# shuwang127/SRCNN_Cpp

Hardware: AMD Instinct MI355X
Metric: SRCNN Y-channel Mpixels/sec (higher is better)
Workload: dtype f32

## Files before the change

srcnn_cpp_amd/csrc/srcnn_pipeline.hip:

```cpp
#include "srcnn_image.h"

#pragma clang fp contract(off)

namespace srcnn {

__device__ __forceinline__ int descale14(int x) { return (x + (1 << 13)) >> 14; }
__device__ __forceinline__ uint8_t sat8(int v) { return (uint8_t)min(max(v, 0), 255); }

__global__ __launch_bounds__(256) void bgr2ycrcb_kernel(const uint8_t *__restrict__ bgr, long stride, int w, int h,
                                                        uint8_t *__restrict__ planes, long pstride, long ppitch)
{
    const int c = blockIdx.x * 256 + threadIdx.x, r = blockIdx.y;
    if (c >= w || r >= h) return;
    const uint8_t *p = bgr + (long)r * stride + 3L * c;
    const int B = p[0], G = p[1], R = p[2];
    const int Y = descale14(B * 1868 + G * 9617 + R * 4899);
    const long o = (long)r * pstride + c;
    planes[o] = sat8(Y);
    planes[ppitch + o] = sat8(descale14((R - Y) * 11682 + (128 << 14)));
    planes[2 * ppitch + o] = sat8(descale14((B - Y) * 9241 + (128 << 14)));
}

__global__ __launch_bounds__(256) void ycrcb2bgr_kernel(const uint8_t *__restrict__ yp, long ystride,
                                                        const uint8_t *__restrict__ crcb, long pstride, long ppitch,
                                                        int w, int h, uint8_t *__restrict__ bgr, long stride)
{
    const int c = blockIdx.x * 256 + threadIdx.x, r = blockIdx.y;
    if (c >= w || r >= h) return;
    const int Y = yp[(long)r * ystride + c];
    const long o = (long)r * pstride + c;
    const int Cr = crcb[o] - 128, Cb = crcb[ppitch + o] - 128;
    uint8_t *p = bgr + (long)r * stride + 3L * c;
    p[0] = sat8(Y + descale14(Cb * 29049));
    p[1] = sat8(Y + descale14(Cb * -5636 + Cr * -11698));
    p[2] = sat8(Y + descale14(Cr * 22987));
}

__device__ __forceinline__ unsigned vresize_px(int h0, int h1, int h2, int h3, int b0, int b1, int b2, int b3, bool simd)
{
    if (simd) {
        const float sc = 1.0f / (2048.0f * 2048.0f);
        float r = __fmul_rn((float)h3, (float)b3 * sc);
        r = __fadd_rn(__fmul_rn((float)h2, (float)b2 * sc), r);
        r = __fadd_rn(__fmul_rn((float)h1, (float)b1 * sc), r);
        r = __fadd_rn(__fmul_rn((float)h0, (float)b0 * sc), r);
        return sat8(__float2int_rn(r));
    }
    return sat8((h0 * b0 + h1 * b1 + h2 * b2 + h3 * b3 + (1 << 21)) >> 22);
}

__global__ __launch_bounds__(256) void resize_cubic_kernel(const uint8_t *__restrict__ src, long sstride, long spitch,
                                                           int sw, int sh, uint8_t *__restrict__ dst, long dstride,
                                                           long dpitch, int dw, int dh,
                                                           const int *__restrict__ xofs, const short *__restrict__ alpha,
                                                           const int *__restrict__ yofs, const short *__restrict__ beta)
{
    const int dx = blockIdx.x * 256 + threadIdx.x, dy = blockIdx.y;
    if (dx >= dw || dy >= dh) return;
    const uint8_t *s = src + (long)blockIdx.z * spitch;
    const int x0 = xofs[dx] - 1, y0 = yofs[dy] - 1;
    int a[4], xs[4];
#pragma unroll
    for (int k = 0; k < 4; ++k) {
        a[k] = alpha[4 * dx + k];
        xs[k] = min(max(x0 + k, 0), sw - 1);
    }
    int hs[4];
#pragma unroll
    for (int ky = 0; ky < 4; ++ky) {
        const uint8_t *row = s + (long)min(max(y0 + ky, 0), sh - 1) * sstride;
        int t = 0;
#pragma unroll
        for (int kx = 0; kx < 4; ++kx) t += row[xs[kx]] * a[kx];
        hs[ky] = t;
    }
    const short *b = beta + 4 * dy;
    dst[(long)blockIdx.z * dpitch + (long)dy * dstride + dx] =
        (uint8_t)vresize_px(hs[0], hs[1], hs[2], hs[3], b[0], b[1], b[2], b[3], dx < dw - dw % 8);
}


__global__ __launch_bounds__(256) void resize_cubic_tiled_kernel(const uint8_t *__restrict__ src, long sstride,
                                                                 long spitch, int sw, int sh,
                                                                 uint8_t *__restrict__ dst, long dstride, long dpitch,
                                                                 int dw, int dh, const int *__restrict__ xofs,
                                                                 const short *__restrict__ alpha,
                                                                 const int *__restrict__ yofs,
                                                                 const short *__restrict__ beta)
{
    __shared__ int hbuf[RMAX][256];
    __shared__ uint8_t sbuf[RMAX][SMAX];
    const int dx0 = blockIdx.x * 256, dx = dx0 + threadIdx.x;
    const int dy0 = blockIdx.y * RT, dy1 = min(dy0 + RT, dh);
    const uint8_t *s = src + (long)blockIdx.z * spitch;
    const int r_lo = yofs[dy0] - 1, r_hi = yofs[dy1 - 1] + 2;
    const int c_lo = xofs[dx0] - 1, c_hi = xofs[min(dx0 + 255, dw - 1)] + 2;
    const int ncol = c_hi - c_lo + 1, nrow = r_hi - r_lo + 1;
    for (int e = threadIdx.x; e < nrow * ncol; e += 256) {
        const int rr = e / ncol, cc = e - rr * ncol;
        sbuf[rr][cc] = s[(long)min(max(r_lo + rr, 0), sh - 1) * sstride + min(max(c_lo + cc, 0), sw - 1)];
    }
    __syncthreads();
    const int dxc = min(dx, dw - 1);
    const int x0 = xofs[dxc] - 1 - c_lo;
    int a[4];
#pragma unroll
    for (int k = 0; k < 4; ++k) a[k] = alpha[4 * dxc + k];
    for (int rr = 0; rr < nrow; ++rr) {
        int t = 0;
#pragma unroll
        for (int k = 0; k < 4; ++k) t += sbuf[rr][x0 + k] * a[k];
        hbuf[rr][threadIdx.x] = t;
    }
    if (dx >= dw) return;
    for (int dy = dy0; dy < dy1; ++dy) {
        const int j = yofs[dy] - 1 - r_lo;
        const short *b = beta + 4 * dy;
        dst[(long)blockIdx.z * dpitch + (long)dy * dstride + dx] =
            (uint8_t)vresize_px(hbuf[j][threadIdx.x], hbuf[j + 1][threadIdx.x], hbuf[j + 2][threadIdx.x],
                                hbuf[j + 3][threadIdx.x], b[0], b[1], b[2], b[3], dx < dw - dw % 8);
    }
}

__device__ __forceinline__ unsigned vpass4(const float (*hbuf)[256], int tx, int j, const short *__restrict__ b, int dx, int dw)
{
    typedef float f32x4 __attribute__((ext_vector_type(4)));
    f32x4 h[4];
#pragma unroll
    for (int k = 0; k < 4; ++k) h[k] = *reinterpret_cast<const f32x4 *>(&hbuf[j + k][4 * tx]);
    unsigned r = 0;
    if (dx + 3 < dw - dw % 8) {
        const float sc = 1.0f / (2048.0f * 2048.0f);
        const float b0 = (float)b[0] * sc, b1 = (float)b[1] * sc, b2 = (float)b[2] * sc, b3 = (float)b[3] * sc;
#pragma unroll
        for (int c = 0; c < 4; ++c) {
            float v = __fmul_rn(h[3][c], b3);
            v = __fadd_rn(__fmul_rn(h[2][c], b2), v);
            v = __fadd_rn(__fmul_rn(h[1][c], b1), v);
            v = __fadd_rn(__fmul_rn(h[0][c], b0), v);
            r |= (unsigned)sat8(__float2int_rn(v)) << (8 * c);
        }
    } else {
#pragma unroll
        for (int c = 0; c < 4; ++c)
            r |= vresize_px((int)h[0][c], (int)h[1][c], (int)h[2][c], (int)h[3][c], b[0], b[1], b[2], b[3], dx + c < dw - dw % 8) << (8 * c);
    }
    return r;
}


__global__ __launch_bounds__(256) void resize_cubic_tiled4_kernel(const uint8_t *__restrict__ src, long sstride,
                                                                  long spitch, int sw, int sh,
                                                                  uint8_t *__restrict__ dst, long dstride, long dpitch,
                                                                  int dw, int dh, const int *__restrict__ xofs,
                                                                  const short *__restrict__ alpha,
                                                                  const int *__restrict__ yofs,
                                                                  const short *__restrict__ beta)
{
    __shared__ __attribute__((aligned(16))) float hbuf[RMAX4][256];
    __shared__ uint8_t sbuf[RMAX4][SMAX];
    const int tid = threadIdx.x;
    const int dx0 = blockIdx.x * 256;
    const int dy0 = blockIdx.y * RT4, dy1 = min(dy0 + RT4, dh);
    const uint8_t *s = src + (long)blockIdx.z * spitch;
    const int r_lo = yofs[dy0] - 1, r_hi = yofs[dy1 - 1] + 2;
    const int c_lo = xofs[dx0] - 1, c_hi = xofs[min(dx0 + 255, dw - 1)] + 2;
    const int ncol = c_hi - c_lo + 1, nrow = r_hi - r_lo + 1;
    for (int e = tid; e < nrow * ncol; e += 256) {
        const int rr = e / ncol, cc = e - rr * ncol;
        sbuf[rr][cc] = s[(long)min(max(r_lo + rr, 0), sh - 1) * sstride + min(max(c_lo + cc, 0), sw - 1)];
    }
    __syncthreads();
    {
        const int dxc = min(dx0 + tid, dw - 1);
        const int x0 = xofs[dxc] - 1 - c_lo;
        int a[4];
#pragma unroll
        for (int k = 0; k < 4; ++k) a[k] = alpha[4 * dxc + k];
        for (int rr = 0; rr < nrow; ++rr) {
            int t = 0;
#pragma unroll
            for (int k = 0; k < 4; ++k) t += sbuf[rr][x0 + k] * a[k];
            hbuf[rr][tid] = (float)t;
        }
    }
    __syncthreads();
    const int tx = tid & 63, ty = tid >> 6;
    const int dx = dx0 + 4 * tx;
    if (dx >= dw) return;
    for (int r = 0; r < RPT; ++r) {
        const int dy = dy0 + RPT * ty + r;
        if (dy >= dy1) break;
        const unsigned v = vpass4(hbuf, tx, yofs[dy] - 1 - r_lo, beta + 4 * dy, dx, dw);
        uint8_t *o = dst + (long)blockIdx.z * dpitch + (long)dy * dstride + dx;
        if (dx + 3 < dw) *reinterpret_cast<unsigned *>(o) = v;
        else
            for (int c = 0; c < 4 && dx + c < dw; ++c) o[c] = (uint8_t)(v >> (8 * c));
    }
}

__device__ __forceinline__ int bgr_to_comp(const uint8_t *px, int comp)
{
    const int B = px[0], G = px[1], R = px[2];
    const int Y = descale14(B * 1868 + G * 9617 + R * 4899);
    if (comp == 0) return sat8(Y);
    if (comp == 1) return sat8(descale14((R - Y) * 11682 + (128 << 14)));
    return sat8(descale14((B - Y) * 9241 + (128 << 14)));
}

struct TileGeom {
    int dx0, dy0, dy1, r_lo, c_lo, ncol, nrow;
};

__device__ __forceinline__ void stage_and_hpass(const uint8_t *__restrict__ bgr, long stride, int sw, int sh, int dw, int comp,
                                                const TileGeom &g, const int *__restrict__ xofs,
                                                const short *__restrict__ alpha, uint8_t (*sbuf)[SMAX], float (*hbuf)[256])
{
    const int tid = threadIdx.x;
    for (int e = tid; e < g.nrow * g.ncol; e += 256) {
        const int rr = e / g.ncol, cc = e - rr * g.ncol;
        sbuf[rr][cc] = (uint8_t)bgr_to_comp(bgr + (long)min(max(g.r_lo + rr, 0), sh - 1) * stride + 3L * min(max(g.c_lo + cc, 0), sw - 1), comp);
    }
    __syncthreads();
    const int dxc = min(g.dx0 + tid, dw - 1);
    const int x0 = xofs[dxc] - 1 - g.c_lo;
    int a[4];
#pragma unroll
    for (int k = 0; k < 4; ++k) a[k] = alpha[4 * dxc + k];
    for (int rr = 0; rr < g.nrow; ++rr) {
        int t = 0;
#pragma unroll
        for (int k = 0; k < 4; ++k) t += sbuf[rr][x0 + k] * a[k];
        hbuf[rr][tid] = (float)t;
    }
    __syncthreads();
}

__device__ __forceinline__ TileGeom tile_geom(int dw, int dh, const int *__restrict__ xofs, const int *__restrict__ yofs)
{
    TileGeom g;
    g.dx0 = blockIdx.x * 256;
    g.dy0 = blockIdx.y * RT4;
    g.dy1 = min(g.dy0 + RT4, dh);
    g.r_lo = yofs[g.dy0] - 1;
    g.c_lo = xofs[g.dx0] - 1;
    g.ncol = xofs[min(g.dx0 + 255, dw - 1)] + 2 - g.c_lo + 1;
    g.nrow = yofs[g.dy1 - 1] + 2 - g.r_lo + 1;
    return g;
}

__global__ __launch_bounds__(256) void bgr_to_y_resized_kernel(const uint8_t *__restrict__ bgr, long stride, int sw, int sh,
                                                               uint8_t *__restrict__ dst, long dstride, int dw, int dh,
                                                               const int *__restrict__ xofs, const short *__restrict__ alpha,
                                                               const int *__restrict__ yofs, const short *__restrict__ beta)
{
    __shared__ __attribute__((aligned(16))) float hbuf[RMAX4][256];
    __shared__ uint8_t sbuf[RMAX4][SMAX];
    const TileGeom g = tile_geom(dw, dh, xofs, yofs);
    stage_and_hpass(bgr, stride, sw, sh, dw, 0, g, xofs, alpha, sbuf, hbuf);
    const int tx = threadIdx.x & 63, ty = threadIdx.x >> 6, dx = g.dx0 + 4 * tx;
    if (dx >= dw) return;
    for (int r = 0; r < RPT; ++r) {
        const int dy = g.dy0 + RPT * ty + r;
        if (dy >= g.dy1) break;
        const unsigned v = vpass4(hbuf, tx, yofs[dy] - 1 - g.r_lo, beta + 4 * dy, dx, dw);
        uint8_t *o = dst + (long)dy * dstride + dx;
        if (dx + 3 < dw) *reinterpret_cast<unsigned *>(o) = v;
        else
            for (int c = 0; c < 4 && dx + c < dw; ++c) o[c] = (uint8_t)(v >> (8 * c));
    }
}

__global__ __launch_bounds__(256) void resize_merge_kernel(const uint8_t *__restrict__ bgr, long stride, int sw, int sh,
                                                           const uint8_t *__restrict__ ysr, long ystride,
                                                           uint8_t *__restrict__ out, long ostride, int dw, int dh,
                                                           const int *__restrict__ xofs, const short *__restrict__ alpha,
                                                           const int *__restrict__ yofs, const short *__restrict__ beta)
{
    __shared__ __attribute__((aligned(16))) float hbuf[RMAX4][256];
    __shared__ uint8_t sbuf[RMAX4][SMAX];
    const TileGeom g = tile_geom(dw, dh, xofs, yofs);
    const int tx = threadIdx.x & 63, ty = threadIdx.x >> 6, dx = g.dx0 + 4 * tx;
    unsigned crcb[2][RPT];
#pragma unroll
    for (int pl = 0; pl < 2; ++pl) {
        if (pl) __syncthreads();
        stage_and_hpass(bgr, stride, sw, sh, dw, 1 + pl, g, xofs, alpha, sbuf, hbuf);
#pragma unroll
        for (int r = 0; r < RPT; ++r) {
            const int dy = min(g.dy0 + RPT * ty + r, g.dy1 - 1);
            crcb[pl][r] = vpass4(hbuf, tx, yofs[dy] - 1 - g.r_lo, beta + 4 * dy, min(dx, dw - 1), dw);
        }
    }
    if (dx >= dw) return;
#pragma unroll
    for (int r = 0; r < RPT; ++r) {
        const int dy = g.dy0 + RPT * ty + r;
        if (dy >= g.dy1) break;
        const uint8_t *yrow = ysr + (long)dy * ystride + dx;
        uint8_t *o = out + (long)dy * ostride + 3L * dx;
        const bool vec = dx + 3 < dw;
        unsigned yv = 0;
        if (vec) yv = *reinterpret_cast<const unsigned *>(yrow);
        else
            for (int c = 0; c < 4 && dx + c < dw; ++c) yv |= (unsigned)yrow[c] << (8 * c);
        uint8_t px[12];
#pragma unroll
        for (int c = 0; c < 4; ++c) {
            const int Y = (yv >> (8 * c)) & 255, Cr = (int)((crcb[0][r] >> (8 * c)) & 255) - 128,
                      Cb = (int)((crcb[1][r] >> (8 * c)) & 255) - 128;
            px[3 * c + 0] = sat8(Y + descale14(Cb * 29049));
            px[3 * c + 1] = sat8(Y + descale14(Cb * -5636 + Cr * -11698));
            px[3 * c + 2] = sat8(Y + descale14(Cr * 22987));
        }
        if (vec) {
            unsigned *o4 = reinterpret_cast<unsigned *>(o);
#pragma unroll
            for (int q = 0; q < 3; ++q)
                o4[q] = px[4 * q] | (px[4 * q + 1] << 8) | (px[4 * q + 2] << 16) | ((unsigned)px[4 * q + 3] << 24);
        } else {
            for (int c = 0; c < 4 && dx + c < dw; ++c)
                for (int q = 0; q < 3; ++q) o[3 * c + q] = px[3 * c + q];
        }
    }
}

bool fused_pipeline_ok(int sw, int sh, int dw, int dh, const void *y_hi, long ystride, const void *out, long ostride)
{
    const bool aligned = ((reinterpret_cast<uintptr_t>(y_hi) | (uintptr_t)ystride | reinterpret_cast<uintptr_t>(out) | (uintptr_t)ostride) & 3) == 0;
    return resize_variant(sw, sh, dw, dh, aligned) == RESIZE_TILED4;
}

hipError_t launch_bgr_to_y_resized(const uint8_t *bgr, long stride, int sw, int sh, uint8_t *dst, long dstride, int dw, int dh,
                                   const int *xofs, const short *alpha, const int *yofs, const short *beta, hipStream_t st)
{
    hipLaunchKernelGGL(bgr_to_y_resized_kernel, dim3((dw + 255) / 256, (dh + RT4 - 1) / RT4), dim3(256), 0, st, bgr, stride, sw,
                       sh, dst, dstride, dw, dh, xofs, alpha, yofs, beta);
    return hipGetLastError();
}

hipError_t launch_resize_merge(const uint8_t *bgr, long stride, int sw, int sh, const uint8_t *ysr, long ystride, uint8_t *out,
                               long ostride, int dw, int dh, const int *xofs, const short *alpha, const int *yofs,
                               const short *beta, hipStream_t st)
{
    hipLaunchKernelGGL(resize_merge_kernel, dim3((dw + 255) / 256, (dh + RT4 - 1) / RT4), dim3(256), 0, st, bgr, stride, sw, sh,
                       ysr, ystride, out, ostride, dw, dh, xofs, alpha, yofs, beta);
    return hipGetLastError();
}

__global__ __launch_bounds__(256) void copy_rows_kernel(uint8_t *__restrict__ dst, long dstride, const uint8_t *__restrict__ src,
                                                        long sstride, int width)
{
    const int x = (blockIdx.x * 256 + threadIdx.x) * 4;
    if (x >= width) return;
    const uint8_t *s = src + (long)blockIdx.y * sstride + x;
    uint8_t *d = dst + (long)blockIdx.y * dstride + x;
    if (x + 4 <= width && (((size_t)s | (size_t)d) & 3) == 0) {
        *reinterpret_cast<unsigned *>(d) = *reinterpret_cast<const unsigned *>(s);
    } else {
        for (int b = 0; b < 4 && x + b < width; ++b) d[b] = s[b];
    }
}

static bool u8_grid_ok(long y, long z = 1) { return y <= kMaxGridYZ && z <= kMaxGridYZ; }

hipError_t launch_copy_rows(uint8_t *dst, long dstride, const uint8_t *src, long sstride, int width, int rows, hipStream_t st)
{
    if (width <= 0 || rows <= 0) return hipSuccess;
    if (!u8_grid_ok(rows)) return hipErrorInvalidValue;
    hipLaunchKernelGGL(copy_rows_kernel, dim3((unsigned)((width + 1023) / 1024), (unsigned)rows), dim3(256), 0, st, dst, dstride, src,
                       sstride, width);
    return hipGetLastError();
}

hipError_t launch_bgr2ycrcb(const uint8_t *bgr, long stride, int w, int h, uint8_t *planes, long pstride,
                            long ppitch, hipStream_t st)
{
    if (!u8_grid_ok(h)) return hipErrorInvalidValue;
    hipLaunchKernelGGL(bgr2ycrcb_kernel, dim3((w + 255) / 256, h), dim3(256), 0, st, bgr, stride, w, h, planes,
                       pstride, ppitch);
    return hipGetLastError();
}

hipError_t launch_ycrcb2bgr(const uint8_t *y, long ystride, const uint8_t *crcb, long pstride, long ppitch, int w,
                            int h, uint8_t *bgr, long stride, hipStream_t st)
{
    if (!u8_grid_ok(h)) return hipErrorInvalidValue;
    hipLaunchKernelGGL(ycrcb2bgr_kernel, dim3((w + 255) / 256, h), dim3(256), 0, st, y, ystride, crcb, pstride,
                       ppitch, w, h, bgr, stride);
    return hipGetLastError();
}

hipError_t launch_resize_cubic(const uint8_t *src, long sstride, long spitch, int sw, int sh, uint8_t *dst,
                               long dstride, long dpitch, int dw, int dh, int n_planes, const int *xofs,
                               const short *alpha, const int *yofs, const short *beta, hipStream_t st)
{
    const bool dword_ok = ((reinterpret_cast<uintptr_t>(dst) | (uintptr_t)dstride | (uintptr_t)dpitch) & 3) == 0;
    const int variant = resize_variant(sw, sh, dw, dh, dword_ok);
    if (!u8_grid_ok(resize_grid_rows(variant, dh), n_planes)) return hipErrorInvalidValue;
    if (variant == RESIZE_TILED4)
        hipLaunchKernelGGL(resize_cubic_tiled4_kernel, dim3((dw + 255) / 256, (dh + RT4 - 1) / RT4, n_planes), dim3(256),
                           0, st, src, sstride, spitch, sw, sh, dst, dstride, dpitch, dw, dh, xofs, alpha, yofs, beta);
    else if (variant == RESIZE_TILED)
        hipLaunchKernelGGL(resize_cubic_tiled_kernel, dim3((dw + 255) / 256, (dh + RT - 1) / RT, n_planes), dim3(256),
                           0, st, src, sstride, spitch, sw, sh, dst, dstride, dpitch, dw, dh, xofs, alpha, yofs, beta);
    else
        hipLaunchKernelGGL(resize_cubic_kernel, dim3((dw + 255) / 256, dh, n_planes), dim3(256), 0, st, src, sstride,
                           spitch, sw, sh, dst, dstride, dpitch, dw, dh, xofs, alpha, yofs, beta);
    return hipGetLastError();
}

typedef float f32x4 __attribute__((ext_vector_type(4)));

__device__ __forceinline__ float cubic_sum4(float s0, float s1, float s2, float s3, const f32x4 c)
{
    float r = __fmul_rn(s0, c[0]);
    r = __fadd_rn(r, __fmul_rn(s1, c[1]));
    r = __fadd_rn(r, __fmul_rn(s2, c[2]));
    return __fadd_rn(r, __fmul_rn(s3, c[3]));
}

struct F32ResizeArgs {
    const float *src;
    long sstride, sch_pitch, sframe_pitch;
    int sw, sh;
    float *dst;
    long dstride, dch_pitch, dframe_pitch;
    int dw, dh;
    int channels, n_planes;
    const int *xfirst, *yfirst;
    const float *xcoef, *ycoef;
};

__global__ __launch_bounds__(256) void resize_cubic_f32_direct_kernel(const F32ResizeArgs p)
{
    const int dx = blockIdx.x * 256 + threadIdx.x;
    if (dx >= p.dw) return;
    const int x0 = p.xfirst[dx] - 1;
    int xs[4];
#pragma unroll
    for (int k = 0; k < 4; ++k) xs[k] = min(max(x0 + k, 0), p.sw - 1);
    const f32x4 a = *reinterpret_cast<const f32x4 *>(p.xcoef + 4L * dx);
    for (int z = blockIdx.z; z < p.n_planes; z += gridDim.z) {
        const int frame = z / p.channels, ch = z - frame * p.channels;
        const float *s = p.src + frame * p.sframe_pitch + ch * p.sch_pitch;
        float *d = p.dst + frame * p.dframe_pitch + ch * p.dch_pitch;
        for (int dy = blockIdx.y; dy < p.dh; dy += gridDim.y) {
            const int y0 = p.yfirst[dy] - 1;
            float hs[4];
#pragma unroll
            for (int ky = 0; ky < 4; ++ky) {
                const float *row = s + (long)min(max(y0 + ky, 0), p.sh - 1) * p.sstride;
                hs[ky] = cubic_sum4(row[xs[0]], row[xs[1]], row[xs[2]], row[xs[3]], a);
            }
            d[(long)dy * p.dstride + dx] = cubic_sum4(hs[0], hs[1], hs[2], hs[3], *reinterpret_cast<const f32x4 *>(p.ycoef + 4L * dy));
        }
    }
}


struct F32LumaArgs {
    float w0, w1, w2, off;
    float g, lo, hi;
    int clamp;
    const float *ysr, *yup;
    long ysr_stride, ysr_frame_pitch, yup_stride, yup_frame_pitch;
};

struct F32TileCols {
    int c_lo, ncol;
    int x0;
    f32x4 a;
    int tx, ty, dx;
};

__device__ __forceinline__ F32TileCols f32_tile_cols(const F32ResizeArgs &p)
{
    F32TileCols t;
    const int tid = threadIdx.x;
    const int dx0 = blockIdx.x * 256;
    t.c_lo = p.xfirst[dx0] - 1;
    const int c_hi = p.xfirst[min(dx0 + 255, p.dw - 1)] + 2;
    t.ncol = c_hi - t.c_lo + 1;
    const int dxc = min(dx0 + tid, p.dw - 1);
    t.x0 = p.xfirst[dxc] - 1 - t.c_lo;
    t.a = *reinterpret_cast<const f32x4 *>(p.xcoef + 4L * dxc);
    t.tx = tid & 63;
    t.ty = tid >> 6;
    t.dx = dx0 + 4 * t.tx;
    return t;
}

template <bool LUMA>
__device__ __forceinline__ void f32_tile_fill(float (*sbuf)[F32_SMAX], const float *s, const F32ResizeArgs &p, const F32LumaArgs &q,
                                              int r_lo, int nrow, int c_lo, int ncol)
{
    for (int e = threadIdx.x; e < nrow * ncol; e += 256) {
        const int rr = e / ncol, cc = e - rr * ncol;
        const long at = (long)min(max(r_lo + rr, 0), p.sh - 1) * p.sstride + min(max(c_lo + cc, 0), p.sw - 1);
        if (LUMA) {
            float y = __fadd_rn(__fmul_rn(q.w0, s[at]), __fmul_rn(q.w1, s[at + p.sch_pitch]));
            y = __fadd_rn(y, __fmul_rn(q.w2, s[at + 2 * p.sch_pitch]));
            sbuf[rr][cc] = __fadd_rn(y, q.off);
        } else {
            sbuf[rr][cc] = s[at];
        }
    }
}

__device__ __forceinline__ void f32_tile_hpass(float (*hbuf)[256], const float (*sbuf)[F32_SMAX], int nrow, const F32TileCols t)
{
    for (int rr = 0; rr < nrow; ++rr)
        hbuf[rr][threadIdx.x] = cubic_sum4(sbuf[rr][t.x0], sbuf[rr][t.x0 + 1], sbuf[rr][t.x0 + 2], sbuf[rr][t.x0 + 3], t.a);
}

__device__ __forceinline__ f32x4 f32_load4(const float *o, int n)
{
    if (n >= 4 && (reinterpret_cast<uintptr_t>(o) & 15) == 0) return *reinterpret_cast<const f32x4 *>(o);
    f32x4 v = {0.f, 0.f, 0.f, 0.f};
#pragma unroll
    for (int c = 0; c < 4; ++c)
        if (c < n) v[c] = o[c];
    return v;
}

template <bool MERGE>
__device__ __forceinline__ void f32_tile_vpass(const float (*hbuf)[256], float *d, const F32ResizeArgs &p, const F32LumaArgs &q,
                                               const f32x4 *add, int dy0, int dy1, int r_lo, const F32TileCols t)
{
    if (t.dx < p.dw) {
#pragma unroll
        for (int r = 0; r < F32_RPT; ++r) {
            const int dy = dy0 + F32_RPT * t.ty + r;
            if (dy >= dy1) break;
            const int j = p.yfirst[dy] - 1 - r_lo;
            const f32x4 b = *reinterpret_cast<const f32x4 *>(p.ycoef + 4L * dy);
            f32x4 h[4];
#pragma unroll
            for (int k = 0; k < 4; ++k) h[k] = *reinterpret_cast<const f32x4 *>(&hbuf[j + k][4 * t.tx]);
            f32x4 v;
#pragma unroll
            for (int c = 0; c < 4; ++c) v[c] = cubic_sum4(h[0][c], h[1][c], h[2][c], h[3][c], b);
            if (MERGE) {
#pragma unroll
                for (int c = 0; c < 4; ++c) {
                    float m = __fadd_rn(v[c], add[r][c]);
                    if (q.clamp) {
                        m = m < q.lo ? q.lo : m;
                        m = m > q.hi ? q.hi : m;
                    }
                    v[c] = m;
                }
            }
            float *o = d + (long)dy * p.dstride + t.dx;
            if (t.dx + 3 < p.dw && (reinterpret_cast<uintptr_t>(o) & 15) == 0) {
                *reinterpret_cast<f32x4 *>(o) = v;
            } else {
#pragma unroll
                for (int c = 0; c < 4; ++c)
                    if (t.dx + c < p.dw) o[c] = v[c];
            }
        }
    }
}

template <bool LUMA>
__device__ __forceinline__ void resize_f32_tiled(const F32ResizeArgs p, const F32LumaArgs q, float (*hbuf)[256],
                                                 float (*sbuf)[F32_SMAX])
{
    const F32TileCols t = f32_tile_cols(p);
    const int n_row_tiles = (p.dh + F32_RT - 1) / F32_RT;
    for (int z = blockIdx.z; z < p.n_planes; z += gridDim.z) {
        const int frame = z / p.channels, ch = z - frame * p.channels;
        const float *s = p.src + frame * p.sframe_pitch + ch * p.sch_pitch;
        float *d = p.dst + frame * p.dframe_pitch + ch * p.dch_pitch;
        for (int rt = blockIdx.y; rt < n_row_tiles; rt += gridDim.y) {
            const int dy0 = rt * F32_RT, dy1 = min(dy0 + F32_RT, p.dh);
            const int r_lo = p.yfirst[dy0] - 1, r_hi = p.yfirst[dy1 - 1] + 2;
            const int nrow = r_hi - r_lo + 1;
            f32_tile_fill<LUMA>(sbuf, s, p, q, r_lo, nrow, t.c_lo, t.ncol);
            __syncthreads();
            f32_tile_hpass(hbuf, sbuf, nrow, t);
            __syncthreads();
            f32_tile_vpass<false>(hbuf, d, p, q, nullptr, dy0, dy1, r_lo, t);
        }
    }
}

__global__ __launch_bounds__(256) void resize_cubic_f32_tiled_kernel(const F32ResizeArgs p)
{
    __shared__ __attribute__((aligned(16))) float hbuf[F32_RMAX][256];
    __shared__ float sbuf[F32_RMAX][F32_SMAX];
    resize_f32_tiled<false>(p, F32LumaArgs{}, hbuf, sbuf);
}

__global__ __launch_bounds__(256) void luma_resize_f32_kernel(const F32ResizeArgs p, const F32LumaArgs q)
{
    __shared__ __attribute__((aligned(16))) float hbuf[F32_RMAX][256];
    __shared__ float sbuf[F32_RMAX][F32_SMAX];
    resize_f32_tiled<true>(p, q, hbuf, sbuf);
}

__global__ __launch_bounds__(256) void resize_merge_f32_kernel(const F32ResizeArgs p, const F32LumaArgs q)
{
    __shared__ __attribute__((aligned(16))) float hbuf[F32_RMAX][256];
    __shared__ float sbuf[F32_RMAX][F32_SMAX];
    const F32TileCols t = f32_tile_cols(p);
    const int n_row_tiles = (p.dh + F32_RT - 1) / F32_RT;
    for (int z = blockIdx.z; z < p.n_planes; z += gridDim.z) {
        const float *s = p.src + z * p.sframe_pitch;
        float *d = p.dst + z * p.dframe_pitch;
        const float *ysr = q.ysr + z * q.ysr_frame_pitch, *yup = q.yup + z * q.yup_frame_pitch;
// ... 651 lines not shown
```

Measured before the change: 8817.

## Vectorize BGR tile staging and compute both chroma planes in one pass

Replaces the per-byte BGR gather with 16-byte vector loads realigned via alignbyte, each thread converting four pixels per group. The merge kernel now reads the source tile once, computing Cr and Cb together and holding Cb in registers until the second horizontal pass, where it previously staged the tile twice. Tap coefficients and tile bounds are loaded once per thread and broadcast with readlane, per-row vertical taps are cached in shared memory, and the Y-plane reads are hoisted ahead of staging to overlap latency. In exchange it adds register pressure and more complex boundary fallback paths.

Measured after the change: 8797. Within noise of the previous version (-0.2%).

```diff
diff --git a/srcnn_cpp_amd/csrc/srcnn_pipeline.hip b/srcnn_cpp_amd/csrc/srcnn_pipeline.hip
--- a/srcnn_cpp_amd/csrc/srcnn_pipeline.hip
+++ b/srcnn_cpp_amd/csrc/srcnn_pipeline.hip
@@ -199,54 +199,168 @@
     }
 }
 
-__device__ __forceinline__ int bgr_to_comp(const uint8_t *px, int comp)
-{
-    const int B = px[0], G = px[1], R = px[2];
-    const int Y = descale14(B * 1868 + G * 9617 + R * 4899);
-    if (comp == 0) return sat8(Y);
-    if (comp == 1) return sat8(descale14((R - Y) * 11682 + (128 << 14)));
-    return sat8(descale14((B - Y) * 9241 + (128 << 14)));
-}
-
 struct TileGeom {
     int dx0, dy0, dy1, r_lo, c_lo, ncol, nrow;
 };
 
-__device__ __forceinline__ void stage_and_hpass(const uint8_t *__restrict__ bgr, long stride, int sw, int sh, int dw, int comp,
-                                                const TileGeom &g, const int *__restrict__ xofs,
-                                                const short *__restrict__ alpha, uint8_t (*sbuf)[SMAX], float (*hbuf)[256])
-{
+typedef unsigned u32x2_a2 __attribute__((ext_vector_type(2), aligned(2)));
+struct TileTaps {
+    int xo, yo, bound;
+    u32x2_a2 a, b;
+};
+
+__device__ __forceinline__ TileTaps tile_taps(int dw, int dh, const int *__restrict__ xofs, const short *__restrict__ alpha,
+                                              const int *__restrict__ yofs, const short *__restrict__ beta)
+{
+    TileTaps t;
     const int tid = threadIdx.x;
-    for (int e = tid; e < g.nrow * g.ncol; e += 256) {
-        const int rr = e / g.ncol, cc = e - rr * g.ncol;
-        sbuf[rr][cc] = (uint8_t)bgr_to_comp(bgr + (long)min(max(g.r_lo + rr, 0), sh - 1) * stride + 3L * min(max(g.c_lo + cc, 0), sw - 1), comp);
-    }
-    __syncthreads();
-    const int dxc = min(g.dx0 + tid, dw - 1);
-    const int x0 = xofs[dxc] - 1 - g.c_lo;
-    int a[4];
-#pragma unroll
-    for (int k = 0; k < 4; ++k) a[k] = alpha[4 * dxc + k];
-    for (int rr = 0; rr < g.nrow; ++rr) {
-        int t = 0;
-#pragma unroll
-        for (int k = 0; k < 4; ++k) t += sbuf[rr][x0 + k] * a[k];
-        hbuf[rr][tid] = (float)t;
-    }
-    __syncthreads();
-}
-
-__device__ __forceinline__ TileGeom tile_geom(int dw, int dh, const int *__restrict__ xofs, const int *__restrict__ yofs)
+    const int dx0 = blockIdx.x * 256, dy0 = blockIdx.y * RT4;
+    const int which = tid & 3;
+    const int *bp = which == 0 ? yofs + dy0 : which == 1 ? xofs + dx0 : which == 2 ? xofs + min(dx0 + 255, dw - 1)
+                                                                                    : yofs + min(dy0 + RT4, dh) - 1;
+    t.bound = *bp;
+    const int dxc = min(dx0 + tid, dw - 1);
+    t.xo = xofs[dxc];
+    t.a = *reinterpret_cast<const u32x2_a2 *>(alpha + 4 * dxc);
+    t.yo = 0;
+    t.b = u32x2_a2{0u, 0u};
+    if (tid < RT4) {
+        const int dyc = min(dy0 + tid, dh - 1);
+        t.yo = yofs[dyc];
+        t.b = *reinterpret_cast<const u32x2_a2 *>(beta + 4 * dyc);
+    }
+    return t;
+}
+
+__device__ __forceinline__ int coef16(const u32x2_a2 v, int k) { return (int)(short)(v[k >> 1] >> (16 * (k & 1))); }
+
+__device__ __forceinline__ TileGeom tile_geom(int dh, const TileTaps &t)
 {
     TileGeom g;
     g.dx0 = blockIdx.x * 256;
     g.dy0 = blockIdx.y * RT4;
     g.dy1 = min(g.dy0 + RT4, dh);
-    g.r_lo = yofs[g.dy0] - 1;
-    g.c_lo = xofs[g.dx0] - 1;
-    g.ncol = xofs[min(g.dx0 + 255, dw - 1)] + 2 - g.c_lo + 1;
-    g.nrow = yofs[g.dy1 - 1] + 2 - g.r_lo + 1;
+    g.r_lo = __builtin_amdgcn_readlane(t.bound, 0) - 1;
+    g.c_lo = __builtin_amdgcn_readlane(t.bound, 1) - 1;
+    g.ncol = __builtin_amdgcn_readlane(t.bound, 2) + 2 - g.c_lo + 1;
+    g.nrow = __builtin_amdgcn_readlane(t.bound, 3) + 2 - g.r_lo + 1;
     return g;
+}
+
+struct __attribute__((aligned(8))) RowTab {
+    short b[RT4][4];
+    int j[RT4];
+};
+
+__device__ __forceinline__ void fill_row_tab(RowTab &tab, const TileTaps &t, int r_lo)
+{
+    const int tid = threadIdx.x;
+    if (tid < RT4) {
+        tab.j[tid] = t.yo - 1 - r_lo;
+#pragma unroll
+        for (int k = 0; k < 4; ++k) tab.b[tid][k] = (short)coef16(t.b, k);
+    }
+}
+
+constexpr int NGRP = SMAX / 4;
+constexpr int NUNIT = (RMAX4 * NGRP + 255) / 256;
+static_assert(SMAX % 4 == 0, "a group is one dword of an sbuf row");
+typedef unsigned u32x4_a4 __attribute__((ext_vector_type(4), aligned(4)));
+
+__device__ __forceinline__ unsigned sat8_descale14(int x) { return (unsigned)min(max(x + (1 << 13), 0), (256 << 14) - 1) >> 14; }
+
+__device__ __forceinline__ int byte12(const unsigned (&w)[3], int n) { return (w[n >> 2] >> (8 * (n & 3))) & 255; }
+
+template <bool CHROMA>
+__device__ __forceinline__ void stage_tile(const uint8_t *__restrict__ bgr, long stride, int sw, int sh, const TileGeom &g,
+                                           uint8_t (*sbuf)[SMAX], int (&at)[NUNIT], unsigned (&later)[NUNIT])
+{
+    const int ngrp = (g.ncol + 3) >> 2;
+    const int q256 = 256 / ngrp, r256 = 256 - q256 * ngrp;
+    int rr = threadIdx.x / ngrp, gc = threadIdx.x - rr * ngrp;
+    const uintptr_t lo = reinterpret_cast<uintptr_t>(bgr);
+    const uintptr_t end = lo + (uintptr_t)((long)(sh - 1) * stride + 3L * sw);
+    unsigned d[NUNIT][4];
+    int sft[NUNIT];
+#pragma unroll
+    for (int i = 0; i < NUNIT; ++i) {
+        at[i] = -1;
+        sft[i] = -1;
+#pragma unroll
+        for (int k = 0; k < 4; ++k) d[i][k] = 0;
+        if (rr < g.nrow) {
+            at[i] = rr * SMAX + 4 * gc;
+            const int col0 = g.c_lo + 4 * gc;
+            const long off = (long)min(max(g.r_lo + rr, 0), sh - 1) * stride + 3L * col0;
+            const uintptr_t a = lo + (uintptr_t)off, a4 = a & ~(uintptr_t)3;
+            if (col0 >= 0 && col0 + 3 < sw && a4 >= lo && a4 + 16 <= end) {
+                const u32x4_a4 v = *reinterpret_cast<const u32x4_a4 *>(bgr + (off - (long)(a & 3)));
+#pragma unroll
+                for (int k = 0; k < 4; ++k) d[i][k] = v[k];
+                sft[i] = (int)(a & 3);
+            }
+        }
+        rr += q256;
+        gc += r256;
+        if (gc >= ngrp) {
+            gc -= ngrp;
+            ++rr;
+        }
+    }
+#pragma unroll
+    for (int i = 0; i < NUNIT; ++i) {
+        if (at[i] >= 0 && sft[i] < 0) {
+            const int r = at[i] / SMAX, c0 = g.c_lo + at[i] - r * SMAX;
+            const uint8_t *row = bgr + (long)min(max(g.r_lo + r, 0), sh - 1) * stride;
+            unsigned b[12];
+#pragma unroll
+            for (int k = 0; k < 4; ++k) {
+                const uint8_t *px = row + 3L * min(max(c0 + k, 0), sw - 1);
+                b[3 * k] = px[0];
+                b[3 * k + 1] = px[1];
+                b[3 * k + 2] = px[2];
+            }
+#pragma unroll
+            for (int q = 0; q < 3; ++q) d[i][q] = b[4 * q] | (b[4 * q + 1] << 8) | (b[4 * q + 2] << 16) | (b[4 * q + 3] << 24);
+            sft[i] = 0;
+        }
+    }
+#pragma unroll
+    for (int i = 0; i < NUNIT; ++i) {
+        later[i] = 0;
+        if (at[i] >= 0) {
+            unsigned w[3];
+#pragma unroll
+            for (int q = 0; q < 3; ++q) w[q] = __builtin_amdgcn_alignbyte(d[i][q + 1], d[i][q], (unsigned)sft[i]);
+            unsigned first = 0, second = 0;
+#pragma unroll
+            for (int k = 0; k < 4; ++k) {
+                const int B = byte12(w, 3 * k), G = byte12(w, 3 * k + 1), R = byte12(w, 3 * k + 2);
+                const int Y = descale14(B * 1868 + G * 9617 + R * 4899);
+                if (CHROMA) {
+                    first |= sat8_descale14((R - Y) * 11682 + (128 << 14)) << (8 * k);
+                    second |= sat8_descale14((B - Y) * 9241 + (128 << 14)) << (8 * k);
+                } else {
+                    first |= (unsigned)sat8(Y) << (8 * k);
+                }
+            }
+            *reinterpret_cast<unsigned *>(&sbuf[0][0] + at[i]) = first;
+            later[i] = second;
+        }
+    }
+}
+
+__device__ __forceinline__ void hpass_tile(const uint8_t (*sbuf)[SMAX], float (*hbuf)[256], int nrow, int x0, const u32x2_a2 taps)
+{
+    int a[4];
+#pragma unroll
+    for (int k = 0; k < 4; ++k) a[k] = coef16(taps, k);
+    for (int rr = 0; rr < nrow; ++rr) {
+        int t = 0;
+#pragma unroll
+        for (int k = 0; k < 4; ++k) t += sbuf[rr][x0 + k] * a[k];
+        hbuf[rr][threadIdx.x] = (float)t;
+    }
 }
 
 __global__ __launch_bounds__(256) void bgr_to_y_resized_kernel(const uint8_t *__restrict__ bgr, long stride, int sw, int sh,
@@ -255,15 +369,24 @@
                                                                const int *__restrict__ yofs, const short *__restrict__ beta)
 {
     __shared__ __attribute__((aligned(16))) float hbuf[RMAX4][256];
-    __shared__ uint8_t sbuf[RMAX4][SMAX];
-    const TileGeom g = tile_geom(dw, dh, xofs, yofs);
-    stage_and_hpass(bgr, stride, sw, sh, dw, 0, g, xofs, alpha, sbuf, hbuf);
+    __shared__ __attribute__((aligned(4))) uint8_t sbuf[RMAX4][SMAX];
+    __shared__ RowTab tab;
+    const TileTaps taps = tile_taps(dw, dh, xofs, alpha, yofs, beta);
+    const TileGeom g = tile_geom(dh, taps);
+    int at[NUNIT];
+    unsigned later[NUNIT];
+    stage_tile<false>(bgr, stride, sw, sh, g, sbuf, at, later);
+    fill_row_tab(tab, taps, g.r_lo);
+    __syncthreads();
+    hpass_tile(sbuf, hbuf, g.nrow, taps.xo - 1 - g.c_lo, taps.a);
+    __syncthreads();
     const int tx = threadIdx.x & 63, ty = threadIdx.x >> 6, dx = g.dx0 + 4 * tx;
     if (dx >= dw) return;
+#pragma unroll
     for (int r = 0; r < RPT; ++r) {
         const int dy = g.dy0 + RPT * ty + r;
         if (dy >= g.dy1) break;
-        const unsigned v = vpass4(hbuf, tx, yofs[dy] - 1 - g.r_lo, beta + 4 * dy, dx, dw);
+        const unsigned v = vpass4(hbuf, tx, tab.j[RPT * ty + r], tab.b[RPT * ty + r], dx, dw);
         uint8_t *o = dst + (long)dy * dstride + dx;
         if (dx + 3 < dw) *reinterpret_cast<unsigned *>(o) = v;
         else
@@ -278,36 +401,60 @@
                                                            const int *__restrict__ yofs, const short *__restrict__ beta)
 {
     __shared__ __attribute__((aligned(16))) float hbuf[RMAX4][256];
-    __shared__ uint8_t sbuf[RMAX4][SMAX];
-    const TileGeom g = tile_geom(dw, dh, xofs, yofs);
-    const int tx = threadIdx.x & 63, ty = threadIdx.x >> 6, dx = g.dx0 + 4 * tx;
+    __shared__ __attribute__((aligned(4))) uint8_t sbuf[RMAX4][SMAX];
+    __shared__ RowTab tab;
+    const TileTaps taps = tile_taps(dw, dh, xofs, alpha, yofs, beta);
+    const int tx = threadIdx.x & 63, ty = threadIdx.x >> 6, dx = (int)blockIdx.x * 256 + 4 * tx;
+    const int dy_first = (int)blockIdx.y * RT4 + RPT * ty;
+    const bool vec = dx + 3 < dw;
+    unsigned yv[RPT];
+#pragma unroll
+    for (int r = 0; r < RPT; ++r) {
+        yv[r] = 0;
+        if (dx < dw && dy_first + r < dh) {
+            const uint8_t *yrow = ysr + (long)(dy_first + r) * ystride + dx;
+            if (vec) yv[r] = *reinterpret_cast<const unsigned *>(yrow);
+            else
+                for (int c = 0; c < 4 && dx + c < dw; ++c) yv[r] |= (unsigned)yrow[c] << (8 * c);
+        }
+    }
+    const TileGeom g = tile_geom(dh, taps);
+    int at[NUNIT];
+    unsigned cb[NUNIT];
+    stage_tile<true>(bgr, stride, sw, sh, g, sbuf, at, cb);
+    fill_row_tab(tab, taps, g.r_lo);
+    const int x0 = taps.xo - 1 - g.c_lo;
+    const int lr_last = g.dy1 - 1 - g.dy0;
     unsigned crcb[2][RPT];
-#pragma unroll
-    for (int pl = 0; pl < 2; ++pl) {
-        if (pl) __syncthreads();
-        stage_and_hpass(bgr, stride, sw, sh, dw, 1 + pl, g, xofs, alpha, sbuf, hbuf);
-#pragma unroll
-        for (int r = 0; r < RPT; ++r) {
-            const int dy = min(g.dy0 + RPT * ty + r, g.dy1 - 1);
-            crcb[pl][r] = vpass4(hbuf, tx, yofs[dy] - 1 - g.r_lo, beta + 4 * dy, min(dx, dw - 1), dw);
-        }
+    __syncthreads();
+    hpass_tile(sbuf, hbuf, g.nrow, x0, taps.a);
+    __syncthreads();
+#pragma unroll
+    for (int i = 0; i < NUNIT; ++i)
+        if (at[i] >= 0) *reinterpret_cast<unsigned *>(&sbuf[0][0] + at[i]) = cb[i];
+#pragma unroll
+    for (int r = 0; r < RPT; ++r) {
+        const int lr = min(RPT * ty + r, lr_last);
+        crcb[0][r] = vpass4(hbuf, tx, tab.j[lr], tab.b[lr], min(dx, dw - 1), dw);
+    }
+    __syncthreads();
+    hpass_tile(sbuf, hbuf, g.nrow, x0, taps.a);
+    __syncthreads();
+#pragma unroll
+    for (int r = 0; r < RPT; ++r) {
+        const int lr = min(RPT * ty + r, lr_last);
+        crcb[1][r] = vpass4(hbuf, tx, tab.j[lr], tab.b[lr], min(dx, dw - 1), dw);
     }
     if (dx >= dw) return;
 #pragma unroll
     for (int r = 0; r < RPT; ++r) {
-        const int dy = g.dy0 + RPT * ty + r;
+        const int dy = dy_first + r;
         if (dy >= g.dy1) break;
-        const uint8_t *yrow = ysr + (long)dy * ystride + dx;
         uint8_t *o = out + (long)dy * ostride + 3L * dx;
-        const bool vec = dx + 3 < dw;
-        unsigned yv = 0;
-        if (vec) yv = *reinterpret_cast<const unsigned *>(yrow);
-        else
-            for (int c = 0; c < 4 && dx + c < dw; ++c) yv |= (unsigned)yrow[c] << (8 * c);
         uint8_t px[12];
 #pragma unroll
         for (int c = 0; c < 4; ++c) {
-            const int Y = (yv >> (8 * c)) & 255, Cr = (int)((crcb[0][r] >> (8 * c)) & 255) - 128,
+            const int Y = (yv[r] >> (8 * c)) & 255, Cr = (int)((crcb[0][r] >> (8 * c)) & 255) - 128,
                       Cb = (int)((crcb[1][r] >> (8 * c)) & 255) - 128;
             px[3 * c + 0] = sat8(Y + descale14(Cb * 29049));
             px[3 * c + 1] = sat8(Y + descale14(Cb * -5636 + Cr * -11698));
```
